# RashmikaDushan/MocapV2

Hardware: NVIDIA B200
Metric: frames/s (detect+match+triangulate, 16-camera 2048x2048 rig, 128 markers) (higher is better)
Workload: dtype u8 (detection, integer exact) / f32 (geometry)

## Files before the change

mocapv2_b200/csrc/detect_cluster.cu:

```cuda
#include "common.cuh"
#include "remap.cuh"
#include "walk.cuh"
#include "tma.cuh"

#define CL_THREADS 128
#ifndef BORDERS_MIN_CTAS
#define BORDERS_MIN_CTAS 1
#endif
#ifndef PF_WIN_L2_PROMO
#define PF_WIN_L2_PROMO 64
#endif
#ifndef BF_THREADS
#define BF_THREADS 128
#endif
#define HOT_MAX 1024
#define CELLS_MAX 8192
#define ROOTS_MAX 512
#define PIECE 64
#define WIN_H 78
#define WIN_H_LOW 56
#define CAND_PER_FRAME 512

#define CN_CLUSTERS 0
#define CN_PIECES 1
// ... 674 lines not shown
            packed_stage_c1(S, pd);
            __syncthreads();
            packed_stage_c2(S, pd, out, wpr);
        } else {
            for (int r = wy; r < uh; r += NWARP)
                for (int c = lane; c < bw; c += 32) {
                    const uint8_t* up = &S.U[r * UW + c];
                    S.HS[r * HSW + c] = (uint16_t)(up[0] + up[1] + up[2] + up[3] + up[4]);
                }
            __syncthreads();
            piece_threshold_majority<false>(S, px0, py0, mw, mh, W, H, T, out, wpr);
        }
        if (s_next >= total) break;
        slot ^= 1;
    }
}

__device__ __forceinline__ void emit_candidate(const ClusterWs& cw, int cid, int f, const short* memb, int m_cnt, int cx, int r, int cty, int cx0, int cy0)
{
    int ax = cx + cx0, ay = r + cy0;
    bool own = false;
    for (int m = 0; m < m_cnt && !own; ++m)
        own = ax >= memb[4 * m] && ax <= memb[4 * m + 2] && ay >= memb[4 * m + 1] && ay <= memb[4 * m + 3];
    if (!own) return;
    int slot = atomicAdd(&cw.cand_count[f], 1);
    if (slot >= CAND_PER_FRAME) { cw.need_general[f] = 7; return; }
    int* e = cw.cand_list + 2 * ((size_t)f * CAND_PER_FRAME + slot);
    e[0] = cid;
    e[1] = cx | (r << 16) | (cty << 31);
}

__device__ __forceinline__ int next_bit(const uint32_t* row, int wpr, int x, uint32_t inv)
{
    int wi = x >> 5;
    uint32_t w = (row[wi] ^ inv) & (~0u << (x & 31));
    while (!w && ++wi < wpr) w = row[wi] ^ inv;
    return w ? wi * 32 + __ffs(w) - 1 : wpr * 32;
}
__device__ __forceinline__ uint32_t range_mask(int wi, int lo, int hi)
{
    int a = max(lo - wi * 32, 0), b = min(hi - wi * 32, 31);
    return (b == 31 ? ~0u : ((1u << (b + 1)) - 1u)) & (~0u << a);
}
__device__ __forceinline__ bool range_any(const uint32_t* row, int lo, int hi)
{
    for (int wi = lo >> 5; wi <= (hi >> 5); ++wi) if (row[wi] & range_mask(wi, lo, hi)) return true;
    return false;
}
__device__ __forceinline__ bool range_all(const uint32_t* row, int lo, int hi)
{
    if (lo > hi) return true;
    for (int wi = lo >> 5; wi <= (hi >> 5); ++wi) { uint32_t m = range_mask(wi, lo, hi); if ((row[wi] & m) != m) return false; }
    return true;
}

__global__ void __launch_bounds__(128) candidates_kernel(ClusterWs cw)
{
    const int lane = threadIdx.x & 31;
    const int warp = (blockIdx.x * blockDim.x + threadIdx.x) >> 5, nwarps = (gridDim.x * blockDim.x) >> 5;
    const int total = min(cw.counters[CN_CLUSTERS], cw.cl_cap);
    int4 ea = make_int4(0, 0, 0, 0), eb = ea;
    if (warp < total) { ea = *(const int4*)(cw.clusters + 8 * (size_t)warp); eb = *(const int4*)(cw.clusters + 8 * (size_t)warp + 4); }
    for (int cid = warp; cid < total; cid += nwarps) {
        const int4 ca = ea, cb = eb;
        if (cid + nwarps < total) {
            ea = *(const int4*)(cw.clusters + 8 * (size_t)(cid + nwarps)); eb = *(const int4*)(cw.clusters + 8 * (size_t)(cid + nwarps) + 4);
        }
        const int f = ca.x;
        const int cx0 = ca.y & 0xffff, cy0 = ca.y >> 16, cx1 = ca.z & 0xffff, cy1 = ca.z >> 16, wpr = cb.x;
        const int mw = cx1 - cx0 + 1, mh = cy1 - cy0 + 1;
        if (mw <= 0 || cw.need_general[f]) continue;
        const int m_off = cb.y & 0xffff, m_cnt = cb.y >> 16;
        const short* memb = cw.memb + ((size_t)f * HOT_MAX + m_off) * 4;
        BitImg im; im.p = cw.rows_out + (unsigned)ca.w; im.W = mw; im.H = mh; im.WPR = wpr;
        for (int r = lane; r < mh; r += 32) {
            const uint32_t* row = im.p + (size_t)r * wpr;
            if (wpr == 2) {
                unsigned long long cur = *(const unsigned long long*)row, up = 0ull;
                if (r > 0) up = *(const unsigned long long*)(row - 2);
                int last_end = -2;
                while (cur) {
                    int s0 = __ffsll((long long)cur) - 1;
                    unsigned long long t = cur >> s0;
                    int len = (~t) ? __ffsll((long long)~t) - 1 : 64;
                    unsigned long long runmask = (len >= 64 ? ~0ull : ((1ull << len) - 1ull)) << s0;
                    cur &= ~runmask;
                    int e0 = s0 + len - 1;
                    unsigned long long dil = runmask | (runmask << 1) | (runmask >> 1);
                    if (last_end >= 0 && r > 0) {
                        unsigned long long gap = ((1ull << s0) - 1ull) & ~((2ull << last_end) - 1ull);
                        if ((up & gap) == gap) emit_candidate(cw, cid, f, memb, m_cnt, last_end, r, 1, cx0, cy0);
                    }
                    if ((up & dil) == 0ull) emit_candidate(cw, cid, f, memb, m_cnt, s0, r, 0, cx0, cy0);
                    last_end = e0;
                }
                continue;
            }
            const uint32_t* above = row - wpr;
            int x = 0, last_end = -2;
            while (x < mw) {
                int s0 = next_bit(row, wpr, x, 0u);
                if (s0 >= mw) break;
                int e1 = min(next_bit(row, wpr, s0, ~0u), mw);
                if (last_end >= 0 && r > 0 && range_all(above, last_end + 1, s0 - 1))
                    emit_candidate(cw, cid, f, memb, m_cnt, last_end, r, 1, cx0, cy0);
                if (r == 0 || !range_any(above, max(s0 - 1, 0), min(e1, mw - 1)))
                    emit_candidate(cw, cid, f, memb, m_cnt, s0, r, 0, cx0, cy0);
                last_end = e1 - 1;
                x = e1;
            }
        }
    }
}

__device__ long long hole_parent_start(const BitImg& im, int lx, int ly, int ox, int oy, int Wabs, int* overflow)
{
    for (int hop = 0; hop < 32; ++hop) {
        int x = lx;
        while (x > 0 && im.get(x - 1, ly)) --x;
        long long mk;
        walk_min_edge(im, x, ly, 4, 1, &mk, overflow);
        if (*overflow) return -1;
        long long pix = mk >> 1;
        int sx = (int)(pix % im.W), sy = (int)(pix / im.W);
        if ((mk & 1) == 0) return (long long)(sy + oy) * Wabs + (sx + ox);
        lx = sx; ly = sy;
    }
    return -1;
}

__device__ void frame_traces(const ClusterWs& cw, int f, int W, int max_contours)
{
    __shared__ int s_holes;
    if (threadIdx.x == 0) s_holes = 0;
    __syncthreads();
    const int n_cand = min(cw.cand_count[f], CAND_PER_FRAME);
    __shared__ uint16_t s_order[CAND_PER_FRAME + 32];
    __shared__ int s_bucket[34];
    if (threadIdx.x < 34) s_bucket[threadIdx.x] = 0;
    __syncthreads();
    auto bucket_of = [&](const int* ce) -> int {
        int mw = (ce[2] & 0xffff) - (ce[1] & 0xffff) + 1, mh = (ce[2] >> 16) - (ce[1] >> 16) + 1;
        bool narrow = ce[4] == 2 && mh <= 1024;
        int b = 15 - min((mw + mh) >> 4, 15);
        return narrow ? 16 + b : b;
    };
    for (int cslot = threadIdx.x; cslot < n_cand; cslot += blockDim.x)
        atomicAdd(&s_bucket[1 + bucket_of(cw.clusters + 8 * (size_t)cw.cand_list[2 * ((size_t)f * CAND_PER_FRAME + cslot)])], 1);
    __syncthreads();
    if (threadIdx.x == 0) {
        int acc = 0;
        for (int b = 1; b <= 32; ++b) { int c = s_bucket[b]; s_bucket[b] = acc; acc += c; if (b == 16) { s_bucket[33] = acc; acc = (acc + 31) & ~31; } }
        s_bucket[0] = acc;
    }
    __syncthreads();
    const int n_wide = s_bucket[33], n_pad = (n_wide + 31) & ~31, n_total = s_bucket[0];
    for (int i = threadIdx.x; i < CAND_PER_FRAME + 32; i += blockDim.x) s_order[i] = 0xffff;
    __syncthreads();
    for (int cslot = threadIdx.x; cslot < n_cand; cslot += blockDim.x) {
        int b = bucket_of(cw.clusters + 8 * (size_t)cw.cand_list[2 * ((size_t)f * CAND_PER_FRAME + cslot)]);
        int pos = atomicAdd(&s_bucket[1 + b], 1);
        s_order[pos] = (uint16_t)cslot;
    }
    __syncthreads();
    for (int base = 0, pass = 0; base < n_total; base += blockDim.x, ++pass) {
        const int it = base + ((pass & 1) ? (int)(blockDim.x - 1 - threadIdx.x) : (int)threadIdx.x);
        if (it >= n_total) continue;
        const int cslot = s_order[it];
        if (cslot == 0xffff) continue;
        const size_t c = (size_t)f * CAND_PER_FRAME + cslot;
        const int* ce = cw.clusters + 8 * (size_t)cw.cand_list[2 * c];
        const int code = cw.cand_list[2 * c + 1];
        const int mx0 = ce[1] & 0xffff, my0 = ce[1] >> 16, mx1 = ce[2] & 0xffff, my1 = ce[2] >> 16;
        const int lx = code & 0xffff, ly = (code >> 16) & 0x7fff, ty = (code >> 31) & 1;
        BitImg im; im.p = cw.rows_out + (unsigned)ce[3]; im.W = mx1 - mx0 + 1; im.H = my1 - my0 + 1; im.WPR = ce[4];
        long long st = (long long)(ly + my0) * W + (lx + mx0);
        long long a[3]; double per; int nch, ovf = 0, bbox[4];
        int ok;
        if (it >= n_pad) ok = trace_contour64<false>(im.p, im.H, 2, 0, im.W, lx, ly, ty ? 0 : 4, 2 * st + ty, a, &per, &nch, &ovf, mx0, my0, W, bbox);
        else if (im.W > 64 && im.H <= 1024) {
            const int wx0 = min(max(lx - 32, 0), im.W - 64);
            ok = trace_contour64<true>(im.p, im.H, im.WPR, wx0, im.W, lx - wx0, ly, ty ? 0 : 4, 2 * st + ty, a, &per, &nch, &ovf, mx0 + wx0, my0, W, bbox);
        } else ok = trace_contour(im, lx, ly, ty ? 0 : 4, 2 * st + ty, a, &per, &nch, &ovf, mx0, my0, W, bbox);
        if (ovf) { cw.need_general[f] = 8; continue; }
        if (!ok) continue;
        long long parent = -1;
        if (ty) {
            parent = hole_parent_start(im, lx, ly, mx0, my0, W, &ovf);
            if (parent < 0) { cw.need_general[f] = 8; continue; }
            atomicAdd(&s_holes, 1);
        }
        int slot = atomicAdd(&cw.rec_count[f], 1);
        if (slot < max_contours) {
            size_t k = (size_t)f * max_contours + slot;
            cw.rec_start[k] = (int)st;
            long long* ra = cw.rec_a + k * 3;
            ra[0] = a[0]; ra[1] = a[1]; ra[2] = a[2];
            cw.rec_per[k] = per;
            int* ri = cw.rec_info + k * 4;
            ri[0] = ty; ri[1] = (int)parent; ri[2] = bbox[0] | (bbox[1] << 16); ri[3] = bbox[2] | (bbox[3] << 16);
        }
    }
    __syncthreads();
    if (s_holes == 0) return;
    const int n = min(cw.rec_count[f], max_contours);
    const int* start = cw.rec_start + (size_t)f * max_contours;
    const int* info = cw.rec_info + (size_t)f * max_contours * 4;
    for (int h = threadIdx.x; h < n; h += blockDim.x) {
        if (!info[4 * h]) continue;
        int x0 = info[4 * h + 2] & 0xffff, y0 = info[4 * h + 2] >> 16, x1 = info[4 * h + 3] & 0xffff, y1 = info[4 * h + 3] >> 16;
        for (int o = 0; o < n; ++o) {
            if (info[4 * o]) continue;
            int ox = start[o] % W, oy = start[o] / W;
            if (ox > x0 && ox < x1 && oy > y0 && oy < y1) { cw.need_general[f] = 9; break; }
        }
    }
}

__device__ void frame_finalize(const ClusterWs& cw, int f, uint8_t* keepv , int max_contours, int max_blobs,
                               double min_area, double min_circ,
                               int32_t* __restrict__ out_xy, int32_t* __restrict__ out_count, int32_t* __restrict__ out_flags,
                               double* __restrict__ out_contours, int32_t* __restrict__ out_contour_count)
{
    const int tid = threadIdx.x;
    const int n = cw.rec_count[f];
    __shared__ int s_kept;
    if (tid == 0) s_kept = 0;
    __syncthreads();
    if (n > max_contours) {
        if (tid == 0) { out_flags[f] |= MOCAP_FLAG_CONTOUR_OVERFLOW; out_count[f] = 0; if (out_contour_count) out_contour_count[f] = 0; }
        return;
    }
    const int* start = cw.rec_start + (size_t)f * max_contours;
    const long long* ra = cw.rec_a + (size_t)f * max_contours * 3;
    const double* rper = cw.rec_per + (size_t)f * max_contours;
    const int* info = cw.rec_info + (size_t)f * max_contours * 4;
    for (int c = tid; c < n; c += (int)blockDim.x) {
        long long a00 = ra[3 * c];
        double area = (double)(a00 < 0 ? -a00 : a00) * 0.5, per = rper[c];
        int keep = 0;
        if (per != 0.0) {
            double circ = __ddiv_rn(__dmul_rn(12.566370614359172, area), __dmul_rn(per, per));
            keep = (circ > min_circ && area > min_area) ? 1 : 0;
        }
        if (a00 == 0) keep = 0;
        keepv[c] = (uint8_t)keep;
    }
    __syncthreads();
    for (int c = tid; c < n; c += (int)blockDim.x) {
        long long a00 = ra[3 * c], a10 = ra[3 * c + 1], a01 = ra[3 * c + 2];
        double per = rper[c];
        int keep = keepv[c];
        const int hole = info[4 * c], st = start[c];
        const int top = hole ? info[4 * c + 1] : st;
        int rank = 0, pos = 0, parent_rank = -1;
        for (int u = 0; u < n; ++u) {
            const int uh = info[4 * u], us = start[u], ut = uh ? info[4 * u + 1] : us;
            bool before;
            if (ut != top) before = ut > top;
            else if (uh != hole) before = !uh;
            else before = us > st;
            rank += before;
            pos += before && keepv[u];
        }
        if (hole) {
            parent_rank = 0;
            for (int u = 0; u < n; ++u) {
                const int uh = info[4 * u], us = start[u], ut = uh ? info[4 * u + 1] : us;
                parent_rank += ut > top;
            }
        }
        if (out_contours && rank < max_contours) {
            double* o = out_contours + ((size_t)f * max_contours + rank) * 8;
            o[0] = (double)a00; o[1] = (double)a10; o[2] = (double)a01; o[3] = per;
            o[4] = (double)hole; o[5] = (double)parent_rank; o[6] = (double)keep; o[7] = (double)st;
        }
        if (!keep) continue;
        atomicAdd(&s_kept, 1);
        if (pos < max_blobs) {
            double sgn = a00 > 0 ? 1.0 : -1.0;
            double m00 = __dmul_rn((double)a00, sgn * 0.5);
            double m10 = __dmul_rn((double)a10, sgn * 0.16666666666666666);
            double m01 = __dmul_rn((double)a01, sgn * 0.16666666666666666);
            out_xy[((size_t)f * max_blobs + pos) * 2 + 0] = (int32_t)__ddiv_rn(m10, m00);
            out_xy[((size_t)f * max_blobs + pos) * 2 + 1] = (int32_t)__ddiv_rn(m01, m00);
        }
    }
    __syncthreads();
    if (tid == 0) {
        int kept = s_kept;
        if (kept > max_blobs) { out_flags[f] |= MOCAP_FLAG_BLOB_OVERFLOW; kept = max_blobs; }
        out_count[f] = kept;
        if (out_contour_count) out_contour_count[f] = n;
    }
}

__global__ void __launch_bounds__(CL_THREADS, BORDERS_MIN_CTAS) borders_finalize_kernel(ClusterWs cw, int W, int frame_step, int max_contours, int max_blobs, double min_area, double min_circ,
                                                                      int32_t* __restrict__ out_xy, int32_t* __restrict__ out_count, int32_t* __restrict__ out_flags,
                                                                      double* __restrict__ out_contours, int32_t* __restrict__ out_contour_count)
{
    DYN_SHARED(smraw);
    const int f = (int)(((long long)blockIdx.x * frame_step) % cw.n_frames);
    if (cw.need_general[f]) return;
    frame_traces(cw, f, W, max_contours);
    __syncthreads();
    if (cw.need_general[f]) return;
    frame_finalize(cw, f, (uint8_t*)smraw, max_contours, max_blobs, min_area, min_circ, out_xy, out_count, out_flags, out_contours, out_contour_count);
}

static int cl_cap_of(int n) { return n * 256 + 1024; }
static int pc_cap_of(int n) { return n * 512 + 2048; }
static size_t rows_cap_of(int n, int H, int W) { size_t w = (size_t)n * ((size_t)H * W / 128 + 4096); return w > 0xf0000000ull ? 0xf0000000ull : w; }

size_t cluster_ws_bytes(int n, int H, int W, int max_contours, ClusterLayout* L)
{
    size_t off = 0;
    auto take = [&](size_t bytes) { size_t r = off; off += align_up(bytes, 256); return r; };
    L->need_general = take((size_t)n * 4);
    L->zero_begin = off;
    L->counters = take(64);
    L->rec_count = take((size_t)n * 4);
    L->cand_count = take((size_t)n * 4);
    L->frame_clusters = take((size_t)n * 8);
    L->zero_bytes = off - L->zero_begin;
    L->clusters = take((size_t)cl_cap_of(n) * 32);
    L->pieces = take((size_t)pc_cap_of(n) * 32);
    L->rec_start = take((size_t)n * max_contours * 4);
    L->rec_a = take((size_t)n * max_contours * 24);
    L->rec_per = take((size_t)n * max_contours * 8);
    L->memb = take((size_t)n * HOT_MAX * 8);
    L->rows_out = take(rows_cap_of(n, H, W) * 4);
    L->cand_list = take((size_t)n * CAND_PER_FRAME * 8);
    L->rec_info = take((size_t)n * max_contours * 16);
    return off;
}

bool cluster_path_supported(int H, int W)
{
    return cdiv(W, TILE) * cdiv(H, TILE) <= CELLS_MAX && W <= 32767 && H <= 32767;
}

int launch_cluster_path(const uint8_t* frames, int n, int H, int W, int64_t fstride, const TableView& tv, int thresh,
                        const uint32_t* cellbox, char* ws_base, const ClusterLayout& L, int* need_general,
                        int max_contours, int max_blobs, double min_area, double min_circ,
                        int32_t* out_xy, int32_t* out_count, int32_t* out_flags, double* out_contours, int32_t* out_contour_count,
                        cudaStream_t s, StageTimer* timer, const ClusterLaunch& how)
{
    ClusterWs cw;
    cw.need_general = need_general;
    cw.counters = (int*)(ws_base + L.counters);
    cw.clusters = (int*)(ws_base + L.clusters);
    cw.pieces = (int*)(ws_base + L.pieces);
    cw.cl_cap = cl_cap_of(n); cw.pc_cap = pc_cap_of(n);
    cw.rec_count = (int*)(ws_base + L.rec_count);
    cw.rec_start = (int*)(ws_base + L.rec_start);
    cw.rec_a = (long long*)(ws_base + L.rec_a);
    cw.rec_per = (double*)(ws_base + L.rec_per);
    cw.memb = (short*)(ws_base + L.memb);
    cw.rows_out = (uint32_t*)(ws_base + L.rows_out);
    cw.rows_cap = (unsigned)rows_cap_of(n, H, W);
    cw.cand_list = (int*)(ws_base + L.cand_list);
    cw.cand_count = (int*)(ws_base + L.cand_count);
    cw.rec_info = (int*)(ws_base + L.rec_info);
    cw.frame_clusters = (int*)(ws_base + L.frame_clusters);
    cw.n_frames = n;
    if (how.zero) CUDA_TRY(cudaMemsetAsync(ws_base + L.zero_begin, 0, L.zero_bytes, s));
    int dev = 0, sms = 148;
    cudaGetDevice(&dev);
    cudaDeviceGetAttribute(&sms, cudaDevAttrMultiProcessorCount, dev);
    const int cells = tv.TX * tv.TY;
    size_t sm_form = (size_t)form_idx_slots(cells) * 2 + (size_t)HOT_MAX * (2 + 4 + 16 + 8 + 8) + (size_t)ROOTS_MAX * (2 + 12) + 64;
#ifndef MOCAP_EMU
    static bool attr_done = false;
    if (!attr_done) { CUDA_TRY(cudaFuncSetAttribute(form_clusters_kernel, cudaFuncAttributeMaxDynamicSharedMemorySize, 64 * 1024)); attr_done = true; }
#endif
    stage_begin(timer, 1, s);
    LAUNCH(form_clusters_kernel, n, CL_THREADS, sm_form, s, cellbox, tv, cw);
    stage_end(timer, 1, s);
    if (how.ev_group) cudaEventRecord(how.ev_group, s);
    stage_begin(timer, 2, s);
#ifdef MOCAP_EMU
    LAUNCH(piece_filter_kernel, sms * how.filter_ctas, CL_THREADS, 0, s, frames, fstride, tv, thresh, cw);
#else
    {
        CUtensorMap tmap, tmap_low;
        memset(&tmap, 0, sizeof(tmap)); memset(&tmap_low, 0, sizeof(tmap_low));
        const int T = thresh + 1;
        const int use_tma = (T >= 0 && T <= 256 && frames_tensor_map(&tmap, frames, n, H, W, fstride, WIN_W, WIN_H, PF_WIN_L2_PROMO) &&
                             frames_tensor_map(&tmap_low, frames, n, H, W, fstride, WIN_W, WIN_H_LOW, PF_WIN_L2_PROMO)) ? 1 : 0;
        LAUNCH(piece_filter_kernel, sms * how.filter_ctas, CL_THREADS, 0, s, frames, fstride, tv, thresh, cw, tmap, tmap_low, use_tma);
    }
#endif
    stage_end(timer, 2, s);
    if (how.ev_filter) cudaEventRecord(how.ev_filter, s);
    stage_begin(timer, 3, s);
    LAUNCH(candidates_kernel, sms * how.cand_ctas, 128, 0, s, cw);
    int frame_step = 1;
    for (int pr : {61, 67, 71, 73}) if (n % pr != 0) { frame_step = pr; break; }
    LAUNCH(borders_finalize_kernel, n, BF_THREADS, (size_t)max_contours + 16, s, cw, W, frame_step, max_contours, max_blobs, min_area, min_circ,
           out_xy, out_count, out_flags, out_contours, out_contour_count);
    stage_end(timer, 3, s);
    if (how.ev_borders) cudaEventRecord(how.ev_borders, s);
    CUDA_TRY(cudaGetLastError());
    return MOCAP_OK;
}
```

mocapv2_b200/csrc/walk.cuh:

```cuda
#pragma once
#include "common.cuh"

struct Walk {
    int x0, y0;
    int x1, y1;
    int x, y;
    int s;
    bool single;
};

__device__ __forceinline__ void walk_init(const BitImg& im, Walk& w, int x, int y, int side)
{
    w.x0 = x; w.y0 = y; w.x = x; w.y = y;
    uint32_t m = im.nbr8(x, y);
    uint32_t rev = __brev(m) >> 24;
    uint32_t sh = (8 - side) & 7;
    uint32_t r = (((rev | (rev << 8)) >> sh) & 0x7fu);
    w.single = r == 0;
    int s = w.single ? (side + 1) & 7 : (side - 1 - (__ffs(r) - 1)) & 7;
    w.s = s;
    w.x1 = x + dir_dx(s); w.y1 = y + dir_dy(s);
}

__device__ __forceinline__ int walk_step(const BitImg& im, Walk& w, unsigned& zeros, bool& done)
{
    uint32_t m = im.nbr8(w.x, w.y);
    int start = (w.s + 1) & 7;
    uint32_t rot = ((m | (m << 8)) >> start) & 0xffu;
    int k = rot ? __ffs(rot) - 1 : 8;
    int d = (start + k) & 7;
    uint32_t z = ((1u << k) - 1u) << start;
    zeros = (z | (z >> 8)) & 0xffu;
    int nx = w.x + dir_dx(d), ny = w.y + dir_dy(d);
    done = (nx == w.x0 && ny == w.y0 && w.x == w.x1 && w.y == w.y1);
    w.x = nx; w.y = ny;
    w.s = (d + 4) & 7;
    return d;
}

#define WALK_BUDGET (1 << 22)

__device__ __forceinline__ long long edge_key(int x, int y, int W, int east) { return 2LL * ((long long)y * W + x) + east; }

static __device__ int walk_min_edge(const BitImg& im, int x, int y, int side, int mode, long long* min_key, int* overflow)
{
    const int W = im.W;
    long long key0 = edge_key(x, y, W, side == 0);
    long long best = key0;
    Walk w; walk_init(im, w, x, y, side);
    if (w.single) { if (min_key) *min_key = edge_key(x, y, W, 0); return side == 4; }
    for (int step = 0; step < WALK_BUDGET; ++step) {
        int cx = w.x, cy = w.y;
        unsigned zeros; bool done;
        walk_step(im, w, zeros, done);
        if (zeros & (1u << 4)) { long long k = edge_key(cx, cy, W, 0); if (k < best) { best = k; if (!mode) return 0; } }
        if (zeros & (1u << 0)) { long long k = edge_key(cx, cy, W, 1); if (k < best) { best = k; if (!mode) return 0; } }
        if (done) { if (min_key) *min_key = best; return best == key0; }
    }
    *overflow = 1;
    if (min_key) *min_key = best;
    return 0;
}

static __device__ int trace_contour(const BitImg& im, int x, int y, int side, long long key0, long long* a, double* per, int* n_chain, int* overflow,
                             int ox, int oy, int Wabs, int* bbox = nullptr)
{
    const int W = Wabs;
    Walk w; walk_init(im, w, x, y, side);
    if (bbox) { bbox[0] = bbox[2] = x + ox; bbox[1] = bbox[3] = y + oy; }
    if (w.single) { a[0] = a[1] = a[2] = 0; *per = 0.0; *n_chain = 1; return key0 < 0 || side == 4; }
    long long a00 = 0, a10 = 0, a01 = 0;
    double perim = 0.0;
    int n = 0;
    int prev_dir = w.s ^ 4;
    bool have_v = false;
    int vx = 0, vy = 0, fx = 0, fy = 0;
    for (int step = 0; step < WALK_BUDGET; ++step) {
        int cx = w.x + ox, cy = w.y + oy;
        unsigned zeros; bool done;
        int d = walk_step(im, w, zeros, done);
        ++n;
        if (key0 >= 0) {
            if ((zeros & (1u << 4)) && edge_key(cx, cy, W, 0) < key0) return 0;
            if ((zeros & (1u << 0)) && edge_key(cx, cy, W, 1) < key0) return 0;
        }
        if (d != prev_dir) {
            if (have_v) {
                long long dxy = (long long)vx * cy - (long long)cx * vy;
                a00 += dxy; a10 += dxy * (vx + cx); a01 += dxy * (vy + cy);
                float ddx = (float)(cx - vx), ddy = (float)(cy - vy);
                perim += (double)__fsqrt_rn(__fadd_rn(__fmul_rn(ddx, ddx), __fmul_rn(ddy, ddy)));
            } else { fx = cx; fy = cy; have_v = true; }
            vx = cx; vy = cy;
            if (bbox) { bbox[0] = min(bbox[0], cx); bbox[1] = min(bbox[1], cy); bbox[2] = max(bbox[2], cx); bbox[3] = max(bbox[3], cy); }
        }
        prev_dir = d;
        if (done) {
            if (have_v) {
                long long dxy = (long long)vx * fy - (long long)fx * vy;
                a00 += dxy; a10 += dxy * (vx + fx); a01 += dxy * (vy + fy);
                float ddx = (float)(fx - vx), ddy = (float)(fy - vy);
                float q = __fadd_rn(__fmul_rn(ddx, ddx), __fmul_rn(ddy, ddy));
                if (q > 0.f) perim += (double)__fsqrt_rn(q);
            }
            a[0] = a00; a[1] = a10; a[2] = a01; *per = perim; *n_chain = n;
            return 1;
        }
    }
    *overflow = 1;
    a[0] = a[1] = a[2] = 0; *per = 0.0; *n_chain = n;
    return 0;
}


template <bool WINDOW>
static __device__ int trace_contour64(const uint32_t* __restrict__ rows, int mh, int wpr, int wx0, int mw, int x, int y, int side, long long key0,
                                      long long* a, double* per, int* n_chain, int* overflow, int ox, int oy, int Wabs, int* bbox)
{
    int wofs = 0;
    int wi0 = wx0 >> 5, wsh = wx0 & 31;
    auto load = [&](int yy) -> unsigned long long {
        if ((unsigned)yy >= (unsigned)mh) return 0ull;
        if (!WINDOW) return *(const unsigned long long*)(rows + 2 * yy);
        const uint32_t* r = rows + (size_t)yy * wpr + wi0;
        const uint32_t w0 = r[0], w1 = r[1], w2 = (wsh && wi0 + 2 < wpr) ? r[2] : 0u;
        const unsigned long long lo = (unsigned long long)w0 | ((unsigned long long)w1 << 32);
        return wsh ? (lo >> wsh) | ((unsigned long long)w2 << (64 - wsh)) : lo;
    };
    auto nbr = [&](unsigned long long up, unsigned long long mid, unsigned long long dn, int xx) -> uint32_t {
        uint32_t u, m, d;
        if (xx) { u = (uint32_t)(up >> (xx - 1)) & 7u; m = (uint32_t)(mid >> (xx - 1)) & 7u; d = (uint32_t)(dn >> (xx - 1)) & 7u; }
        else { u = ((uint32_t)up << 1) & 7u; m = ((uint32_t)mid << 1) & 7u; d = ((uint32_t)dn << 1) & 7u; }
        return ((m >> 2) & 1u) | (((u >> 2) & 1u) << 1) | (((u >> 1) & 1u) << 2) | ((u & 1u) << 3) |
               ((m & 1u) << 4) | ((d & 1u) << 5) | (((d >> 1) & 1u) << 6) | (((d >> 2) & 1u) << 7);
    };
    unsigned long long up = load(y - 1), mid = load(y), dn = load(y + 1);
    if (bbox) { bbox[0] = bbox[2] = x + ox; bbox[1] = bbox[3] = y + oy; }
    uint32_t m0 = nbr(up, mid, dn, x);
    uint32_t rev = __brev(m0) >> 24, sh = (8 - side) & 7;
    uint32_t r0 = (((rev | (rev << 8)) >> sh) & 0x7fu);
    if (r0 == 0) { a[0] = a[1] = a[2] = 0; *per = 0.0; *n_chain = 1; return key0 < 0 || side == 4; }
    int s = (side - 1 - (__ffs(r0) - 1)) & 7;
    const int x0 = x, y0 = y, x1 = x + dir_dx(s), y1 = y + dir_dy(s);
    const int kbase = 2 * (oy * Wabs + ox);
    const int key0i = (int)key0;
    long long a00 = 0, a10 = 0, a01 = 0;
    int axis_len = 0, n_diag1 = 0;
    double perim_long = 0.0;
    int n = 0, prev_dir = s ^ 4;
    bool have_v = false;
    int vx = 0, vy = 0, fx = 0, fy = 0;
    int bx0 = x, bx1 = x, by0 = y, by1 = y;
    int wx = x, wy = y;
    for (int step = 0; step < WALK_BUDGET; ++step) {
        const int cx = wx, cy = wy;
        uint32_t m = nbr(up, mid, dn, wx - wofs);
        int start = (s + 1) & 7;
        uint32_t rot = ((m | (m << 8)) >> start) & 0xffu;
        int k = rot ? __ffs(rot) - 1 : 8;
        int d = (start + k) & 7;
        uint32_t z = ((1u << k) - 1u) << start;
        uint32_t zeros = (z | (z >> 8)) & 0xffu;
        int nx = wx + dir_dx(d), ny = wy + dir_dy(d);
        bool done = (nx == x0 && ny == y0 && wx == x1 && wy == y1);
        bool slide = false;
        if (WINDOW) {
            const int bx = nx - wofs, org = wx0 + wofs;
            slide = (bx == 0 && org > 0) || (bx == 63 && org + 64 < mw);
            if (slide) {
                const int norg = min(max(wx0 + nx - 32, 0), mw - 64);
                wofs = norg - wx0; wi0 = norg >> 5; wsh = norg & 31;
                up = load(ny - 1); mid = load(ny); dn = load(ny + 1);
            }
        }
        if (!slide && ny != wy) {
            const bool goup = ny < wy;
            const unsigned long long nr = load(goup ? ny - 1 : ny + 1), om = mid;
            mid = goup ? up : dn;
            up = goup ? nr : om;
            dn = goup ? om : nr;
        }
        wx = nx; wy = ny; s = (d + 4) & 7;
        ++n;
        if (key0 >= 0 && (zeros & 0x11u)) {
            int kk = kbase + 2 * (cy * Wabs + cx);
            if ((zeros & (1u << 4)) && kk < key0i) return 0;
            if ((zeros & (1u << 0)) && kk + 1 < key0i) return 0;
        }
        if (d != prev_dir) {
            if (have_v) {
                int dxy = vx * cy - cx * vy;
                a00 += dxy;
                if (WINDOW) { a10 += (long long)dxy * (vx + cx); a01 += (long long)dxy * (vy + cy); }
                else { a10 += dxy * (vx + cx); a01 += dxy * (vy + cy); }
                int adx = abs(cx - vx), ady = abs(cy - vy);
                if (adx == 0 || ady == 0) axis_len += adx + ady;
                else if (adx == 1) ++n_diag1;
                else perim_long += (double)__fsqrt_rn((float)(2 * adx * adx));
            } else { fx = cx; fy = cy; have_v = true; }
            vx = cx; vy = cy;
            bx0 = min(bx0, cx); bx1 = max(bx1, cx); by0 = min(by0, cy); by1 = max(by1, cy);
        }
        prev_dir = d;
        if (done) {
            if (have_v) {
                int dxy = vx * fy - fx * vy;
                a00 += dxy;
                if (WINDOW) { a10 += (long long)dxy * (vx + fx); a01 += (long long)dxy * (vy + fy); }
                else { a10 += dxy * (vx + fx); a01 += dxy * (vy + fy); }
                int adx = abs(fx - vx), ady = abs(fy - vy);
                if (adx == 0 || ady == 0) axis_len += adx + ady;
                else if (adx == 1) ++n_diag1;
                else perim_long += (double)__fsqrt_rn((float)(2 * adx * adx));
            }
            a[0] = a00; a[1] = a10 + 3LL * ox * a00; a[2] = a01 + 3LL * oy * a00;
            *per = (double)axis_len + (double)n_diag1 * (double)__fsqrt_rn(2.0f) + perim_long;
            *n_chain = n;
            if (bbox) { bbox[0] = bx0 + ox; bbox[1] = by0 + oy; bbox[2] = bx1 + ox; bbox[3] = by1 + oy; }
            return 1;
        }
    }
    *overflow = 1;
    a[0] = a[1] = a[2] = 0; *per = 0.0; *n_chain = n;
    return 0;
}
```

Before: 732,900.

## Replace contour-walk neighbor logic with shared-memory step lookup table

Builds a 512-entry-by-8-direction lookup table in shared memory that maps a 3x3 neighborhood and the current direction to the next direction, an abandon threshold and the step deltas. The contour tracer then replaces per-step bit gathering and __ffs logic with one table byte read. It also restructures the Green-moment and perimeter accumulation into per-step form with run-length tracking of diagonal runs, and keeps a five-row register window. The cost is building the table once per block and a shared-memory lookup on the serial per-step critical path, and the perimeter and moment bookkeeping is more intricate to get exactly right.

After: 757,400, median of 6. 1.03x the previous value.

```diff
diff --git a/mocapv2_b200/csrc/detect_cluster.cu b/mocapv2_b200/csrc/detect_cluster.cu
--- a/mocapv2_b200/csrc/detect_cluster.cu
+++ b/mocapv2_b200/csrc/detect_cluster.cu
@@ -1000,6 +1000,7 @@
     DYN_SHARED(smraw);
     const int f = (int)(((long long)blockIdx.x * frame_step) % cw.n_frames);
     if (cw.need_general[f]) return;
+    step_table_build();
     frame_traces(cw, f, W, max_contours);
     __syncthreads();
     if (cw.need_general[f]) return;
diff --git a/mocapv2_b200/csrc/walk.cuh b/mocapv2_b200/csrc/walk.cuh
--- a/mocapv2_b200/csrc/walk.cuh
+++ b/mocapv2_b200/csrc/walk.cuh
@@ -22,15 +22,19 @@
     w.x1 = x + dir_dx(s); w.y1 = y + dir_dy(s);
 }
 
-__device__ __forceinline__ int walk_step(const BitImg& im, Walk& w, unsigned& zeros, bool& done)
-{
-    uint32_t m = im.nbr8(w.x, w.y);
-    int start = (w.s + 1) & 7;
+__device__ __forceinline__ int walk_rule(uint32_t m, int s, unsigned& zeros)
+{
+    int start = (s + 1) & 7;
     uint32_t rot = ((m | (m << 8)) >> start) & 0xffu;
     int k = rot ? __ffs(rot) - 1 : 8;
-    int d = (start + k) & 7;
     uint32_t z = ((1u << k) - 1u) << start;
     zeros = (z | (z >> 8)) & 0xffu;
+    return (start + k) & 7;
+}
+
+__device__ __forceinline__ int walk_step(const BitImg& im, Walk& w, unsigned& zeros, bool& done)
+{
+    int d = walk_rule(im.nbr8(w.x, w.y), w.s, zeros);
     int nx = w.x + dir_dx(d), ny = w.y + dir_dy(d);
     done = (nx == w.x0 && ny == w.y0 && w.x == w.x1 && w.y == w.y1);
     w.x = nx; w.y = ny;
@@ -113,114 +117,136 @@
 }
 
 
+#define STEP_TAB_BYTES 4096
+__shared__ uint32_t step_tab[STEP_TAB_BYTES / 4];
+
+__device__ __forceinline__ uint32_t nbr8_of_raw9(uint32_t r)
+{
+    return ((r >> 5) & 1u) | (((r >> 2) & 1u) << 1) | (((r >> 1) & 1u) << 2) | ((r & 1u) << 3) |
+           (((r >> 3) & 1u) << 4) | (((r >> 6) & 1u) << 5) | (((r >> 7) & 1u) << 6) | (((r >> 8) & 1u) << 7);
+}
+
+__device__ __forceinline__ void step_table_build()
+{
+    for (int r = threadIdx.x; r < STEP_TAB_BYTES / 8; r += blockDim.x) {
+        const uint32_t m = nbr8_of_raw9((uint32_t)r);
+        uint32_t w[2] = {0u, 0u};
+#pragma unroll
+        for (int s = 0; s < 8; ++s) {
+            unsigned zeros;
+            const int d = walk_rule(m, s, zeros);
+            const uint32_t thr = (zeros & (1u << 4)) ? 0u : (zeros & 1u) ? 1u : 2u;
+            const uint32_t e = thr | ((uint32_t)(d ^ 4) << 2) | ((dir_dy(d) < 0 ? 1u : 0u) << 5) | ((uint32_t)(dir_dx(d) + 1) << 6);
+            w[s >> 2] |= e << (8 * (s & 3));
+        }
+        step_tab[2 * r] = w[0]; step_tab[2 * r + 1] = w[1];
+    }
+}
+
+__device__ __forceinline__ uint32_t step_index(unsigned long long up, unsigned long long mid, unsigned long long dn, int col1, uint32_t s)
+{
+    const int sh = max(col1, 0);
+    const uint32_t k = col1 < 0 ? 4u : 3u;
+    const uint32_t u = (uint32_t)(up >> sh) << k, m = (uint32_t)(mid >> sh) << (k + 3), d = (uint32_t)(dn >> sh) << (k + 6);
+    return (u & 0x38u) | (m & 0x1c0u) | (d & 0xe00u) | s;
+}
+
+template <bool WINDOW> struct GreenAcc { typedef uint32_t T; };
+template <> struct GreenAcc<true> { typedef long long T; };
+
 template <bool WINDOW>
-static __device__ int trace_contour64(const uint32_t* __restrict__ rows, int mh, int wpr, int wx0, int mw, int x, int y, int side, long long key0,
-                                      long long* a, double* per, int* n_chain, int* overflow, int ox, int oy, int Wabs, int* bbox)
+static __device__ int trace_contour64(const uint32_t* __restrict__ rows, int mh, int wpr, int wx0, int mw,
+                                      int x, int y, int side, long long key0, long long* a, double* per, int* n_chain, int* overflow,
+                                      int ox, int oy, int Wabs, int* bbox)
 {
     int wofs = 0;
     int wi0 = wx0 >> 5, wsh = wx0 & 31;
+    const unsigned long long* rows64 = (const unsigned long long*)rows;
     auto load = [&](int yy) -> unsigned long long {
         if ((unsigned)yy >= (unsigned)mh) return 0ull;
-        if (!WINDOW) return *(const unsigned long long*)(rows + 2 * yy);
+        if (!WINDOW) return rows64[(unsigned)yy];
         const uint32_t* r = rows + (size_t)yy * wpr + wi0;
         const uint32_t w0 = r[0], w1 = r[1], w2 = (wsh && wi0 + 2 < wpr) ? r[2] : 0u;
         const unsigned long long lo = (unsigned long long)w0 | ((unsigned long long)w1 << 32);
         return wsh ? (lo >> wsh) | ((unsigned long long)w2 << (64 - wsh)) : lo;
     };
-    auto nbr = [&](unsigned long long up, unsigned long long mid, unsigned long long dn, int xx) -> uint32_t {
-        uint32_t u, m, d;
-        if (xx) { u = (uint32_t)(up >> (xx - 1)) & 7u; m = (uint32_t)(mid >> (xx - 1)) & 7u; d = (uint32_t)(dn >> (xx - 1)) & 7u; }
-        else { u = ((uint32_t)up << 1) & 7u; m = ((uint32_t)mid << 1) & 7u; d = ((uint32_t)dn << 1) & 7u; }
-        return ((m >> 2) & 1u) | (((u >> 2) & 1u) << 1) | (((u >> 1) & 1u) << 2) | ((u & 1u) << 3) |
-               ((m & 1u) << 4) | ((d & 1u) << 5) | (((d >> 1) & 1u) << 6) | (((d >> 2) & 1u) << 7);
-    };
-    unsigned long long up = load(y - 1), mid = load(y), dn = load(y + 1);
+    unsigned long long u2 = load(y - 2), up = load(y - 1), mid = load(y), dn = load(y + 1), d2 = load(y + 2);
     if (bbox) { bbox[0] = bbox[2] = x + ox; bbox[1] = bbox[3] = y + oy; }
-    uint32_t m0 = nbr(up, mid, dn, x);
+    uint32_t m0 = nbr8_of_raw9(step_index(up, mid, dn, x - 1, 0) >> 3);
     uint32_t rev = __brev(m0) >> 24, sh = (8 - side) & 7;
     uint32_t r0 = (((rev | (rev << 8)) >> sh) & 0x7fu);
     if (r0 == 0) { a[0] = a[1] = a[2] = 0; *per = 0.0; *n_chain = 1; return key0 < 0 || side == 4; }
-    int s = (side - 1 - (__ffs(r0) - 1)) & 7;
-    const int x0 = x, y0 = y, x1 = x + dir_dx(s), y1 = y + dir_dy(s);
-    const int kbase = 2 * (oy * Wabs + ox);
-    const int key0i = (int)key0;
-    long long a00 = 0, a10 = 0, a01 = 0;
-    int axis_len = 0, n_diag1 = 0;
+    const int s0 = (side - 1 - (__ffs(r0) - 1)) & 7;
+    const int lin1 = (y + dir_dy(s0)) * Wabs + x + dir_dx(s0);
+    const int kt = key0 >= 0 ? (int)key0 - 2 * (oy * Wabs + ox) : -(1 << 30);
+    uint32_t a00 = 0;
+    typename GreenAcc<WINDOW>::T a10 = 0, a01 = 0;
+    int n_diag = 0, n_long = 0;
     double perim_long = 0.0;
-    int n = 0, prev_dir = s ^ 4;
-    bool have_v = false;
-    int vx = 0, vy = 0, fx = 0, fy = 0;
+    int s = s0, run = -(1 << 30), first_turn = WALK_BUDGET;
     int bx0 = x, bx1 = x, by0 = y, by1 = y;
     int wx = x, wy = y;
-    for (int step = 0; step < WALK_BUDGET; ++step) {
-        const int cx = wx, cy = wy;
-        uint32_t m = nbr(up, mid, dn, wx - wofs);
-        int start = (s + 1) & 7;
-        uint32_t rot = ((m | (m << 8)) >> start) & 0xffu;
-        int k = rot ? __ffs(rot) - 1 : 8;
-        int d = (start + k) & 7;
-        uint32_t z = ((1u << k) - 1u) << start;
-        uint32_t zeros = (z | (z >> 8)) & 0xffu;
-        int nx = wx + dir_dx(d), ny = wy + dir_dy(d);
-        bool done = (nx == x0 && ny == y0 && wx == x1 && wy == y1);
+    int col1 = x - 1;
+    int n = 0;
+    bool abandon = false, done = false;
+#pragma unroll 1
+    while (n < WALK_BUDGET) {
+        const uint32_t e = ((const uint8_t*)step_tab)[step_index(up, mid, dn, col1, s)];
+        const int sn = (e >> 2) & 7, thr = e & 3;
+        const int dx = (int)(e >> 6) - 1, dy = (e & 0x20u) ? -1 : (e & 0x0cu) ? 1 : 0;
+        const int lin = wy * Wabs + wx;
+        ++n;
+        abandon = thr < 2 && kt - 2 * lin > thr;
+        done = lin == lin1 && sn == s0;
+        const int dxy = wx * dy - dx * wy;
+        a00 += (uint32_t)dxy;
+        if (WINDOW) { a10 += (long long)dxy * (2 * wx + dx); a01 += (long long)dxy * (2 * wy + dy); }
+        else { a10 += (uint32_t)dxy * (uint32_t)(2 * wx + dx); a01 += (uint32_t)dxy * (uint32_t)(2 * wy + dy); }
+        bx0 = min(bx0, wx); bx1 = max(bx1, wx); by0 = min(by0, wy); by1 = max(by1, wy);
+        n_diag += sn & 1;
+        const bool turn = sn != s;
+        if (turn && (s & 1) && run > 1) {
+            perim_long += (double)__fsqrt_rn((float)(2 * run * run));
+            n_long += run;
+        }
+        if (turn) first_turn = min(first_turn, n);
+        run = turn ? 1 : run + 1;
+        s = sn;
+        if (abandon || done) break;
+        const int nx = wx + dx, ny = wy + dy;
+        col1 += dx;
         bool slide = false;
         if (WINDOW) {
-            const int bx = nx - wofs, org = wx0 + wofs;
+            const int bx = col1 + 1, org = wx0 + wofs;
             slide = (bx == 0 && org > 0) || (bx == 63 && org + 64 < mw);
             if (slide) {
                 const int norg = min(max(wx0 + nx - 32, 0), mw - 64);
                 wofs = norg - wx0; wi0 = norg >> 5; wsh = norg & 31;
-                up = load(ny - 1); mid = load(ny); dn = load(ny + 1);
+                col1 = nx - wofs - 1;
+                u2 = load(ny - 2); up = load(ny - 1); mid = load(ny); dn = load(ny + 1); d2 = load(ny + 2);
             }
         }
-        if (!slide && ny != wy) {
-            const bool goup = ny < wy;
-            const unsigned long long nr = load(goup ? ny - 1 : ny + 1), om = mid;
-            mid = goup ? up : dn;
-            up = goup ? nr : om;
-            dn = goup ? om : nr;
-        }
-        wx = nx; wy = ny; s = (d + 4) & 7;
-        ++n;
-        if (key0 >= 0 && (zeros & 0x11u)) {
-            int kk = kbase + 2 * (cy * Wabs + cx);
-            if ((zeros & (1u << 4)) && kk < key0i) return 0;
-            if ((zeros & (1u << 0)) && kk + 1 < key0i) return 0;
-        }
-        if (d != prev_dir) {
-            if (have_v) {
-                int dxy = vx * cy - cx * vy;
-                a00 += dxy;
-                if (WINDOW) { a10 += (long long)dxy * (vx + cx); a01 += (long long)dxy * (vy + cy); }
-                else { a10 += dxy * (vx + cx); a01 += dxy * (vy + cy); }
-                int adx = abs(cx - vx), ady = abs(cy - vy);
-                if (adx == 0 || ady == 0) axis_len += adx + ady;
-                else if (adx == 1) ++n_diag1;
-                else perim_long += (double)__fsqrt_rn((float)(2 * adx * adx));
-            } else { fx = cx; fy = cy; have_v = true; }
-            vx = cx; vy = cy;
-            bx0 = min(bx0, cx); bx1 = max(bx1, cx); by0 = min(by0, cy); by1 = max(by1, cy);
-        }
-        prev_dir = d;
-        if (done) {
-            if (have_v) {
-                int dxy = vx * fy - fx * vy;
-                a00 += dxy;
-                if (WINDOW) { a10 += (long long)dxy * (vx + fx); a01 += (long long)dxy * (vy + fy); }
-                else { a10 += dxy * (vx + fx); a01 += dxy * (vy + fy); }
-                int adx = abs(fx - vx), ady = abs(fy - vy);
-                if (adx == 0 || ady == 0) axis_len += adx + ady;
-                else if (adx == 1) ++n_diag1;
-                else perim_long += (double)__fsqrt_rn((float)(2 * adx * adx));
-            }
-            a[0] = a00; a[1] = a10 + 3LL * ox * a00; a[2] = a01 + 3LL * oy * a00;
-            *per = (double)axis_len + (double)n_diag1 * (double)__fsqrt_rn(2.0f) + perim_long;
-            *n_chain = n;
-            if (bbox) { bbox[0] = bx0 + ox; bbox[1] = by0 + oy; bbox[2] = bx1 + ox; bbox[3] = by1 + oy; }
-            return 1;
-        }
-    }
-    *overflow = 1;
-    a[0] = a[1] = a[2] = 0; *per = 0.0; *n_chain = n;
-    return 0;
-}
+        if (!slide && dy != 0) {
+            const unsigned long long nr = load(ny + 2 * dy);
+            if (dy < 0) { d2 = dn; dn = mid; mid = up; up = u2; u2 = nr; }
+            else { u2 = up; up = mid; mid = dn; dn = d2; d2 = nr; }
+        }
+        wx = nx; wy = ny;
+    }
+    if (!abandon && !done) {
+        *overflow = 1;
+        a[0] = a[1] = a[2] = 0; *per = 0.0; *n_chain = n;
+        return 0;
+    }
+    if (abandon) return 0;
+    const int k = run + first_turn - 1;
+    if ((s0 & 1) && k > 1) { perim_long += (double)__fsqrt_rn((float)(2 * k * k)); n_long += k; }
+    const long long A00 = (int)a00;
+    a[0] = A00;
+    if (WINDOW) { a[1] = a10 + 3LL * ox * A00; a[2] = a01 + 3LL * oy * A00; }
+    else { a[1] = (long long)(int)a10 + 3LL * ox * A00; a[2] = (long long)(int)a01 + 3LL * oy * A00; }
+    *per = (double)(n - n_diag) + (double)(n_diag - n_long) * (double)__fsqrt_rn(2.0f) + perim_long;
+    *n_chain = n;
+    if (bbox) { bbox[0] = bx0 + ox; bbox[1] = by0 + oy; bbox[2] = bx1 + ox; bbox[3] = by1 + oy; }
+    return 1;
+}
```
